# mikestir/webradio

Hardware: AMD Instinct MI355X
Metric: complex Msamples/sec (node), 256-ch DDC+NFM demod (higher is better)
Workload: dtype f32

## Files before the change

webradio_amd/csrc/wr_capi_internal.h:

```cpp
#ifndef WR_CAPI_INTERNAL_H
#define WR_CAPI_INTERNAL_H

#include "wr_internal.h"

#include <cstdarg>
#include <cstdio>
#include <cstdlib>
#include <cstring>
#include <new>
#include <atomic>
#include <chrono>
#include <map>
#include <mutex>
#include <vector>

#define HIP_TRY(expr)                                                                    \
	do {                                                                                 \
		hipError_t e_ = (expr);                                                          \
		if (e_ != hipSuccess)                                                            \
			return wrc_fail(WR_ERR_HIP, "%s: %s (%s:%d)", #expr, hipGetErrorString(e_),  \
			                __FILE__, __LINE__);                                         \
	} while (0)


// ... 130 lines not shown
	std::vector<hipEvent_t> ev;
	size_t ev_used;
	double prof_ms;
	unsigned int prof_n;
	struct RingSlot {
		float *host = nullptr;
		size_t cap = 0;
		hipEvent_t done = nullptr;
		size_t stride = 0, frames = 0;
		unsigned int slots = 0;
		unsigned long long seq = 0;
		unsigned int stream_wait = 0;
		unsigned long long stream_gen = 0;
	};
	std::vector<RingSlot> ring;
	unsigned int ring_head = 0, ring_count = 0;
	bool ring_held = false;
	unsigned long long ring_overruns = 0;
	unsigned long long submit_seq = 0;
	bool defer_post = true;
	unsigned int coalesce = 1;
	const float *held_base = nullptr;
	size_t held_frames = 0, held_each = 0;
	unsigned int held_count = 0;
	std::mutex ring_lock;
	struct Stream {
		bool enabled = false;
		bool host_bytes = false;
		bool live = false;
		bool unchecked = false;
		WrStreamCtl *ctl = nullptr;
		WrStreamDesc *desc = nullptr;
		WrStreamDev *sdev = nullptr;
		float *ring = nullptr;
		size_t ring_floats = 0;
		Group *g = nullptr;
		unsigned int count = 0;
		size_t nframes = 0;
		bool u8 = false;
		int parity0 = 0;
		size_t k1 = 0, k2 = 0;
		unsigned long long gen = 0;
		unsigned long long blocks = 0;
		std::chrono::steady_clock::time_point last_bell;
		const float *last_iq = nullptr;
		uint8_t *raw[4] = {nullptr, nullptr, nullptr, nullptr};
		size_t raw_cap = 0;
		unsigned long long raw_next = 0;
		unsigned long long raw_gen[4] = {0, 0, 0, 0};
		unsigned int raw_idx[4] = {0, 0, 0, 0};
		hipEvent_t raw_ev = nullptr;
		bool ext = false;
		bool up_pending = false;
		unsigned long long host_blocks = 0;
		unsigned long long long_blocks = 0;
	} stream;
};

struct wr_spectrum {
	wr_dev *dev;
	unsigned int n, hop;
	unsigned int ch;
	WrFftPlan plan;
	float *stage;
	size_t stage_cap;
	size_t pending;
// ... 66 lines not shown
```

webradio_amd/csrc/wr_internal.h:

```cpp
#ifndef WR_INTERNAL_H_
#define WR_INTERNAL_H_

#include <hip/hip_runtime.h>
#include <stddef.h>
#include <stdint.h>

#include "webradio_amd.h"

#define WR_HIST      (WR_FIR_LENGTH - 1)
#define WR_LANES     64
#define WR_SPLIT_N   256
#define WR_MAX_DEVICES 64
#define WR_TAPSETS   4

int         wrc_fail(int code, const char *fmt, ...) __attribute__((format(printf, 2, 3)));
int         wrc_dev_index(const wr_dev *dev);
hipStream_t wrc_dev_stream(const wr_dev *dev);
int         wrc_tuner_launch_mark(wr_tuner *t, hipEvent_t *ev);

void     wrd_sin_table(float *table);
void     wrd_sin_table_rounded(float *table);
int      wrd_phase_step(int if_hz, unsigned int input_rate);
unsigned wrd_lowpass_maxbin(unsigned int fir_length, unsigned int passband, unsigned int input_rate);
void     wrd_lowpass_design(unsigned int fir_length, unsigned int passband, unsigned int input_rate, float *coeff);
// ... 130 lines not shown
	unsigned int pad;
};
struct WrStreamCtl {
	volatile unsigned int ready;
	volatile unsigned int stop;
	volatile unsigned int pad0[14];
	volatile unsigned int done;
	volatile unsigned int final_blocks;
	volatile unsigned int err;
	volatile unsigned int self_closed;
	volatile unsigned int long_blocks;
	volatile unsigned int pad1[11];
};
#define WR_STREAM_SHARDS 16u
struct WrStreamDev {
	unsigned int ready, stop;
	unsigned long long beat;
	unsigned int ready_up;
	unsigned int pad0[27];
	unsigned long long progress;
	unsigned int drain_from;
	unsigned int pad1[29];
	unsigned int post_done[WR_STREAM_MAXJ];
	unsigned int post_fine[WR_STREAM_MAXJ];
	unsigned int post_ticket[WR_STREAM_MAXJ];
	unsigned int ddc_done[WR_STREAM_MAXJ][WR_STREAM_SHARDS][32];
	WrStreamDesc desc[WR_STREAM_MAXJ];
	unsigned long long cur[WR_STREAM_MAXJ + 1u];
};
struct WrStreamArgs {
	WrStreamCtl        *ctl;
	const WrStreamDesc *desc_host;
	WrStreamDev        *sdev;
	unsigned long long  idle_ticks;
	unsigned long long  wait_ticks;
	unsigned int        n_ddc, n_post;
	unsigned long long *tl;
	unsigned long long  cur0, audio0;
	unsigned long long  nframes;
	unsigned int        k1, d1, is_u8;
	unsigned int        ext;
	unsigned int        slots, groups;
	unsigned long long  gmap0, gmap1;
	unsigned int        kslow;
	unsigned int        kmax;
	const float        *hist;
	float              *hist_next;
	const unsigned int *phase, *step;
	unsigned int       *phase_next;
	const float        *hist_cs, *hist_lo;
	float              *hist_cs_next, *hist_lo_next;
	const int          *flags;
	const float        *taps1, *rot, *taps1u;
	const int          *tapsel;
	const float        *table, *hi_cs, *lo_cs;
	float              *ring;
	float              *audio_bufs[4];
	WrPostArgs          post;
	unsigned int        drain_run, drain_ntiles;
	const float        *prev_iq[2];
	float              *dem[2];
	int                 parity0;
	unsigned int        one_filter;
};
#define WR_STREAM_ERR_WAIT   1u
hipError_t wrk_stream_geometry(unsigned int d2, unsigned int groups, unsigned int kmax, bool one_filter, unsigned int nseg,
                               int num_cus, unsigned int *n_ddc, unsigned int *n_post);
hipError_t wrk_tuner_stream(hipStream_t st, const WrStreamArgs &A, void *ev_start, void *ev_stop);

struct WrFftPlan {
	unsigned int n;
	unsigned int channels;
	unsigned int n1, n2;
	float *tw_n;
	float *tw_sub;
	float *window;
	float *window_p1;
	float *work;
	size_t work_frames;
};
hipError_t wrk_fft_frames(hipStream_t st, const WrFftPlan &P, const float *iq, size_t hop,
                          size_t nframes_fft, float *bins_out , float *db_out );

hipError_t wrk_fft_cols(hipStream_t st, const WrFftPlan &P, const float *iq, unsigned int S, unsigned int cols, size_t first,
                        float *db, int num_cus );

size_t     wrk_chan_levels_work(unsigned int cols, size_t k1);
hipError_t wrk_chan_levels(hipStream_t st, const float *iq, size_t S, unsigned int cols, size_t k1, unsigned int d2, size_t k2,
                           const float *squelch, float *work, const float **out);

struct WrAgcPar {
	float        target;
// ... 26 lines not shown
```

webradio_amd/csrc/wr_stream_kernel.inc:

```

__device__ __forceinline__ unsigned int st_rfl(unsigned int v) { return __builtin_amdgcn_readfirstlane(v); }
__device__ __forceinline__ unsigned int st_ld(const unsigned int *p)
{
	return st_rfl(__hip_atomic_load(p, __ATOMIC_RELAXED, __HIP_MEMORY_SCOPE_AGENT));
}
__device__ __forceinline__ unsigned long long st_ld64(const unsigned long long *p)
{
	const unsigned long long v = __hip_atomic_load(p, __ATOMIC_RELAXED, __HIP_MEMORY_SCOPE_AGENT);
	return ((unsigned long long)st_rfl((unsigned int)(v >> 32)) << 32) | st_rfl((unsigned int)v);
}
__device__ __forceinline__ unsigned int st_ld_sys(const volatile unsigned int *p)
{
	return st_rfl(__hip_atomic_load((const unsigned int *)p, __ATOMIC_RELAXED, __HIP_MEMORY_SCOPE_SYSTEM));
}
__device__ __forceinline__ void st_st_sys(volatile unsigned int *p, unsigned int v)
{
	__hip_atomic_store((unsigned int *)p, v, __ATOMIC_RELAXED, __HIP_MEMORY_SCOPE_SYSTEM);
}

__device__ __forceinline__ unsigned int st_ddc_ready(const WrStreamArgs &S)
{
	return st_rfl((unsigned int)__hip_atomic_load(&S.sdev->progress, __ATOMIC_RELAXED, __HIP_MEMORY_SCOPE_AGENT));
}
__device__ __forceinline__ unsigned int st_post_ready(const WrStreamArgs &S)
{
	return st_rfl((unsigned int)(__hip_atomic_load(&S.sdev->progress, __ATOMIC_RELAXED, __HIP_MEMORY_SCOPE_AGENT) >> 32));
}

__device__ __forceinline__ void stream_fail(const WrStreamArgs &S)
{
	st_st_sys(&S.ctl->err, WR_STREAM_ERR_WAIT);
	__hip_atomic_store(&S.sdev->stop, 1u, __ATOMIC_RELAXED, __HIP_MEMORY_SCOPE_AGENT);
// ... 26 lines not shown
			if (now - t0 > S.wait_ticks && now >= beat && now - beat > S.wait_ticks) {
				stream_fail(S);
				if (r > known)
					known = r;
				closed = true;
				return false;
			}
		}
		__builtin_amdgcn_s_sleep(20);
	}
}

__device__ __forceinline__ bool stream_wait_count(const WrStreamArgs &S, const unsigned int *p, unsigned int target)
{
	if (st_ld(p) >= target)
		return true;
	const unsigned long long t0 = __builtin_amdgcn_s_memrealtime();
	unsigned int spins = 0;
	for (;;) {
		__builtin_amdgcn_s_sleep(20);
		if (st_ld(p) >= target)
			return true;
		if ((++spins & 63u) == 0u) {
			if (__builtin_amdgcn_s_memrealtime() - t0 > S.wait_ticks) {
				stream_fail(S);
				return false;
			}
			if (st_ld_sys(&S.ctl->err))
				return false;
		}
	}
}

#define STREAM_DRAIN_BLOCKS 2u
__device__ __forceinline__ void stream_watch(const WrStreamArgs &S)
{
	const unsigned int lane = threadIdx.x & 63u;
	__builtin_amdgcn_s_setprio(3);
	const unsigned int units = S.k1 * S.groups;
	unsigned int known = 1, jd = 0, jp = 0;
	unsigned int df = 0;
	unsigned int nlong = 0;
	bool closed = false;
	unsigned long long t_last = __builtin_amdgcn_s_memrealtime();
#ifdef STREAM_TL
	if ((threadIdx.x & 63u) == 0 && S.tl)
		S.tl[6999u * 8u + 0u] = t_last;
#endif
	for (;;) {
		bool moved = false;
		auto look = [&]() __attribute__((always_inline)) {
			const unsigned int r = st_ld(&S.sdev->ready);
			if (r > known)
				known = r;
			if (st_ld(&S.sdev->stop)) {
				const unsigned int f = st_ld(&S.sdev->ready);
				if (f > known)
					known = f;
				closed = true;
				const unsigned int from = known >= STREAM_DRAIN_BLOCKS ? known - STREAM_DRAIN_BLOCKS : 0u;
				df = (jd > from ? jd : from) + 1u;
				__hip_atomic_store(&S.sdev->drain_from, df, __ATOMIC_RELAXED, __HIP_MEMORY_SCOPE_AGENT);
				__builtin_amdgcn_fence(__ATOMIC_RELEASE, "agent");
			}
		};
		if (!closed && (jd >= known || jp >= known))
			look();
		if (jd < known && jd < WR_STREAM_MAXJ) {
			unsigned int v = 0;
			if (lane < WR_STREAM_SHARDS)
				v = __hip_atomic_load(&S.sdev->ddc_done[jd][lane][0], __ATOMIC_RELAXED, __HIP_MEMORY_SCOPE_AGENT);
#pragma unroll
			for (int o = 8; o >= 1; o >>= 1)
				v += __shfl_xor(v, o, 64);
			if (st_rfl(v) >= units) {
				{
					unsigned int fine = 1u;
					if (S.drain_run != S.post.run) {
						if (!closed)
							look();
						fine = (df && jd + 1u >= df) ? 1u : known >= jd + 3u ? 0u : 1u;
					}
					__hip_atomic_store(&S.sdev->post_fine[jd], fine, __ATOMIC_RELAXED, __HIP_MEMORY_SCOPE_AGENT);
					if (!fine && lane == 0)
						st_st_sys(&S.ctl->long_blocks, ++nlong);
					asm volatile("s_waitcnt vmcnt(0)" ::: "memory");
				}
				++jd;
				__hip_atomic_store(&S.sdev->progress, ((unsigned long long)jp << 32) | jd, __ATOMIC_RELAXED, __HIP_MEMORY_SCOPE_AGENT);
				moved = true;
#ifdef STREAM_TL
				if (lane == 0 && S.tl && jd <= 256u)
					S.tl[(7000u + jd - 1u) * 8u + 0u] = __builtin_amdgcn_s_memrealtime();
#endif
			}
		}
		if (jp < jd && st_ld(&S.sdev->post_done[jp]) >= (st_ld(&S.sdev->post_fine[jp]) ? S.drain_ntiles : S.post.ntiles) * S.post.groups) {
			++jp;
			__hip_atomic_store(&S.sdev->progress, ((unsigned long long)jp << 32) | jd, __ATOMIC_RELAXED, __HIP_MEMORY_SCOPE_AGENT);
			if (lane == 0)
				st_st_sys(&S.ctl->done, jp);
			moved = true;
#ifdef STREAM_TL
			if (lane == 0 && S.tl && jp <= 256u)
				S.tl[(7000u + jp - 1u) * 8u + 1u] = __builtin_amdgcn_s_memrealtime();
#endif
		}
		if (closed && jp >= known)
			return;
		const unsigned long long now = __builtin_amdgcn_s_memrealtime();
		if (moved) {
			t_last = now;
		} else {
			if ((jd < known || jp < jd) && now - t_last > S.wait_ticks) {
				stream_fail(S);
				return;
			}
			if (closed && st_ld_sys(&S.ctl->err))
				return;
			__builtin_amdgcn_s_sleep(4);
		}
	}
}

__device__ __forceinline__ void stream_bell(const WrStreamArgs &S)
{
	if (threadIdx.x >= 64u && threadIdx.x < 128u) {
		stream_watch(S);
		return;
	}
	if (threadIdx.x != 0)
		return;
	__builtin_amdgcn_s_setprio(3);
	unsigned int seen = 1;
	__hip_atomic_store(&S.sdev->desc[0].cur, S.cur0, __ATOMIC_RELAXED, __HIP_MEMORY_SCOPE_AGENT);
	__hip_atomic_store(&S.sdev->desc[0].audio_host, S.audio0, __ATOMIC_RELAXED, __HIP_MEMORY_SCOPE_AGENT);
	__hip_atomic_store(&S.sdev->cur[1], S.cur0, __ATOMIC_RELAXED, __HIP_MEMORY_SCOPE_AGENT);
	asm volatile("s_waitcnt vmcnt(0)" ::: "memory");
	unsigned long long t_last = __builtin_amdgcn_s_memrealtime();
	for (;;) {
		__hip_atomic_store(&S.sdev->beat, (unsigned long long)__builtin_amdgcn_s_memrealtime(), __ATOMIC_RELAXED,
		                   __HIP_MEMORY_SCOPE_AGENT);
		const unsigned int s = st_ld_sys(&S.ctl->stop);
		unsigned int r = st_ld_sys(&S.ctl->ready);
		{
			const unsigned int ru = st_ld(&S.sdev->ready_up);
			if (ru > r)
				r = ru;
		}
		if (r > WR_STREAM_MAXJ)
			r = WR_STREAM_MAXJ;
		if (r > seen) {
			for (unsigned int j = seen; j < r; ++j) {
				const unsigned long long c = __hip_atomic_load(&S.desc_host[j].cur, __ATOMIC_RELAXED, __HIP_MEMORY_SCOPE_SYSTEM);
				const unsigned long long a = __hip_atomic_load(&S.desc_host[j].audio_host, __ATOMIC_RELAXED, __HIP_MEMORY_SCOPE_SYSTEM);
				__hip_atomic_store(&S.sdev->desc[j].cur, c, __ATOMIC_RELAXED, __HIP_MEMORY_SCOPE_AGENT);
				__hip_atomic_store(&S.sdev->cur[j + 1u], c, __ATOMIC_RELAXED, __HIP_MEMORY_SCOPE_AGENT);
				__hip_atomic_store(&S.sdev->desc[j].audio_host, a, __ATOMIC_RELAXED, __HIP_MEMORY_SCOPE_AGENT);
			}
			asm volatile("s_waitcnt vmcnt(0)" ::: "memory");
			__hip_atomic_store(&S.sdev->ready, r, __ATOMIC_RELAXED, __HIP_MEMORY_SCOPE_AGENT);
			seen = r;
			t_last = __builtin_amdgcn_s_memrealtime();
		}
		if (s || st_ld(&S.sdev->stop)) {
			asm volatile("s_waitcnt vmcnt(0)" ::: "memory");
			__hip_atomic_store(&S.sdev->stop, 1u, __ATOMIC_RELAXED, __HIP_MEMORY_SCOPE_AGENT);
			return;
		}
		if (seen >= WR_STREAM_MAXJ || __builtin_amdgcn_s_memrealtime() - t_last > S.idle_ticks) {
			if (seen < WR_STREAM_MAXJ)
				st_st_sys(&S.ctl->self_closed, 1u);
			asm volatile("s_waitcnt vmcnt(0)" ::: "memory");
			__hip_atomic_store(&S.sdev->stop, 1u, __ATOMIC_RELAXED, __HIP_MEMORY_SCOPE_AGENT);
			return;
		}
		__builtin_amdgcn_s_sleep(40);
	}
}

template <unsigned int PD2, unsigned int TS, unsigned int NSEG>
__device__ __forceinline__ void stream_post(const WrStreamArgs &S, const unsigned int p, v2f *lds, const bool helper)
{
	constexpr unsigned int D2 = PD2 ? PD2 : 1u;
	constexpr unsigned int NEED = (POST_TK - 1u) * D2 + WR_FIR_LENGTH * NSEG;
	wave_prio(3u);
	if (threadIdx.x >= POST_THREADS)
		return;
	const unsigned int wave = st_rfl(threadIdx.x >> 6);
	const unsigned int waves_per_wg = POST_THREADS / 64u;
#ifdef STREAM_TL
	if (threadIdx.x == 0 && S.tl && !helper)
		S.tl[(6000u + p) * 8u + 7u] = 12345ull;
#endif

	const unsigned int n_bnd = (S.kslow * S.groups + waves_per_wg - 1u) / waves_per_wg;
	if (!helper && p < n_bnd) {
		const unsigned long long c0 = S.cur0;
		ddc_body<WR_NCO_ROTATE, true, PD2>(S.is_u8 ? nullptr : (const float2 *)c0, S.is_u8 ? (const uchar2 *)c0 : nullptr,
		                                   (const float2 *)S.hist, (float2 *)S.hist_next, (size_t)S.nframes, (size_t)S.k1, S.d1,
		                                   S.slots, S.groups, S.phase, S.step, (const float2 *)S.hist_cs, S.flags, S.phase_next,
		                                   (float2 *)S.hist_cs_next, (const float2 *)S.hist_lo, (float2 *)S.hist_lo_next, S.taps1,
		                                   (const float4 *)S.rot, S.taps1u, S.tapsel, TS == 1u ? 1u : S.kmax, (float2 *)S.ring, S.table,
		                                   (const float2 *)S.hi_cs, (const float2 *)S.lo_cs, S.n_ddc, S.post, S.gmap0, S.gmap1, 0,
		                                   S.kslow, 0x40000000u, 0u, 0u, lds, DDC_ROLE_BOUNDARY);
		const unsigned int ub = p * waves_per_wg + wave;
		asm volatile("s_waitcnt vmcnt(0)" ::: "memory");
		if (ub / S.groups < S.kslow && (threadIdx.x & 63u) == 0u)
			__hip_atomic_fetch_add(&S.sdev->ddc_done[0][ub % WR_STREAM_SHARDS][0], 1u, __ATOMIC_RELAXED, __HIP_MEMORY_SCOPE_AGENT);
		wave_prio(3u);
		__syncthreads();
	}

	float *stage = (float *)lds;
	float *tile = stage + NEED * 64u;
	int *modes = (int *)(tile + POST_TK * 65u);
	unsigned int *sh = (unsigned int *)(modes + 64);
	const unsigned int tasks = S.post.ntiles * S.post.groups;
	unsigned int known = 1;
	bool closed = false;
	unsigned int j = 0;
	if (helper) {
		if (threadIdx.x == 0)
			sh[6] = st_ld(&S.sdev->drain_from);
		__syncthreads();
		const unsigned int df = sh[6];
		if (!df)
// ... 10 lines not shown
		if (threadIdx.x == 0) {
			bool ok = j < WR_STREAM_MAXJ && stream_wait_ready(S, j, known, closed);
			if (ok) {
				const unsigned int need_hi = j >= 4u ? j - 3u : 0u;
				const unsigned long long t0 = __builtin_amdgcn_s_memrealtime();
				unsigned int spins = 0;
				for (;;) {
					const unsigned long long pg = st_ld64(&S.sdev->progress);
					if ((unsigned int)pg >= j + 1u && (unsigned int)(pg >> 32) >= need_hi)
						break;
					if ((++spins & 63u) == 0u) {
						if (__builtin_amdgcn_s_memrealtime() - t0 > S.wait_ticks) {
							stream_fail(S);
							ok = false;
							break;
						}
						if (st_ld_sys(&S.ctl->err)) {
							ok = false;
							break;
						}
					}
					__builtin_amdgcn_s_sleep(20);
				}
			}
			unsigned long long ah = 0;
			unsigned int drain = helper ? 1u : 0u;
			if (ok) {
				ah = j ? st_ld64(&S.sdev->desc[j].audio_host) : S.audio0;
				__builtin_amdgcn_fence(__ATOMIC_ACQUIRE, "agent");
				if (!helper) {
					const unsigned int df = st_ld(&S.sdev->drain_from);
					drain = (df && j + 1u >= df) ? 1u : 0u;
				}
				sh[7] = (helper || drain) ? 1u : st_ld(&S.sdev->post_fine[j]);
			}
			sh[5] = drain;
			sh[0] = ok ? 1u : 0u;
			sh[1] = (unsigned int)ah;
			sh[2] = (unsigned int)(ah >> 32);
			sh[3] = known;
		}
		__syncthreads();
		const bool go = sh[0] != 0u;
		const unsigned long long ah = ((unsigned long long)sh[2] << 32) | sh[1];
		known = sh[3];
		if (!go)
			break;
		WrPostArgs A = S.post;
		A.chan_iq = S.ring + (size_t)(j % WR_STREAM_RING) * S.k1 * S.slots * 2u;
		A.chan_prev = j ? S.ring + (size_t)((j - 1u) % WR_STREAM_RING) * S.k1 * S.slots * 2u : nullptr;
		A.prev_iq = S.prev_iq[S.parity0];
		A.dem_hist = S.dem[S.parity0];
		A.audio_host = (float *)ah;
		A.audio = S.audio_bufs[j & 3u];
#ifdef STREAM_TL
		const unsigned long long pt1 = __builtin_amdgcn_s_memtime();
		if (threadIdx.x == 0 && S.tl && !helper && p < 4u && j < 256u)
			S.tl[(7300u + j) * 8u + p * 2u] = __builtin_amdgcn_s_memrealtime();
#endif
		const bool drain = sh[5] != 0u;
		if (sh[7] != 0u) {
			A.run = S.drain_run;
			A.ntiles = S.drain_ntiles;
		}
		const unsigned int tasks_j = A.ntiles * A.groups;
		unsigned int mine = 0;
		const unsigned int rot = (unsigned int)(((unsigned long long)j * tasks) % S.n_post);
		for (unsigned int t = p >= rot ? p - rot : p + S.n_post - rot;; t += S.n_post) {
			if (drain) {
				if (threadIdx.x == 0)
					sh[4] = __hip_atomic_fetch_add(&S.sdev->post_ticket[j], 1u, __ATOMIC_RELAXED, __HIP_MEMORY_SCOPE_AGENT);
				__syncthreads();
				t = sh[4];
			}
			if (t >= tasks_j)
				break;
			post_role<D2, false, NSEG>(A, t % A.ntiles, t / A.ntiles, stage, tile, modes);
			__syncthreads();
			++mine;
		}
		if (threadIdx.x == 0 && mine) {
			if (ah)
				__builtin_amdgcn_fence(__ATOMIC_RELEASE, "");
			else
				__builtin_amdgcn_fence(__ATOMIC_RELEASE, "agent");
			asm volatile("s_waitcnt vmcnt(0)" ::: "memory");
			__hip_atomic_fetch_add(&S.sdev->post_done[j], mine, __ATOMIC_RELAXED, __HIP_MEMORY_SCOPE_AGENT);
		}
#ifdef STREAM_TL
		if (threadIdx.x == 0 && S.tl && !helper && p < 4u && j < 256u)
			S.tl[(7300u + j) * 8u + p * 2u + 1u] = __builtin_amdgcn_s_memrealtime();
		if (threadIdx.x == 0) {
			const unsigned long long pt3 = __builtin_amdgcn_s_memtime();
			pt_wait += pt1 - pt0;
			pt_sync += pt3 - pt1;
			++pt_n;
// ... 331 lines not shown
	return nseg == 1u || nseg == 2u || (nseg == 4u && d2 <= STREAM_NSEG4_MAX_D2);
}
template <unsigned int PD2, class F>
static hipError_t with_stream_nseg(unsigned int nseg, F &&f)
{
	if (nseg == 1u)
		return f(std::integral_constant<unsigned int, 1u>());
	if (nseg == 2u)
		return f(std::integral_constant<unsigned int, 2u>());
	if constexpr (PD2 <= STREAM_NSEG4_MAX_D2)
		if (nseg == 4u)
			return f(std::integral_constant<unsigned int, 4u>());
	return hipErrorInvalidValue;
}

template <unsigned int PD2, unsigned int NG, unsigned int TS, unsigned int NSEG>
static hipError_t stream_allow_lds(size_t lds)
{
	static bool attr_done[WR_MAX_DEVICES];
	if (lds <= 64 * 1024)
		return hipSuccess;
	return allow_lds((const void *)k_tuner_stream<PD2, NG, TS, NSEG>, stream_lds_bytes(PD2, TS, NSEG), attr_done);
}

template <unsigned int PD2, unsigned int NG, unsigned int TS, unsigned int NSEG>
static hipError_t stream_occupancy(size_t lds, int *per_cu)
{
	hipError_t e = stream_allow_lds<PD2, NG, TS, NSEG>(lds);
	if (e != hipSuccess)
		return e;
	return hipOccupancyMaxActiveBlocksPerMultiprocessor(per_cu, k_tuner_stream<PD2, NG, TS, NSEG>, (int)(DDC_ROTATE_WAVES * 64u), lds);
}

hipError_t wrk_stream_geometry(unsigned int d2, unsigned int groups, unsigned int kmax, bool one_filter, unsigned int nseg,
                               int num_cus, unsigned int *n_ddc, unsigned int *n_post)
{
	*n_ddc = *n_post = 0;
	if (!wrk_tuner_post_supported(d2) || !stream_nseg_supported(d2, nseg) || !groups || groups > 16u || !kmax ||
	    kmax > WR_TAPSETS)
		return hipSuccess;
	unsigned int ng, ts;
	stream_shape(groups, kmax, one_filter, &ng, &ts);
	const size_t lds = stream_lds_bytes(d2, ts == 1u ? 1u : kmax, nseg);
	int per_cu = 0;
	hipError_t e = with_post_d2(d2, [&](auto D2) {
		constexpr unsigned int PD2 = decltype(D2)::value;
		return with_stream_nseg<PD2>(nseg, [&](auto NS) {
			constexpr unsigned int NSEG = decltype(NS)::value;
			return ts != 1u ? stream_occupancy<PD2, 1, WR_TAPSETS, NSEG>(lds, &per_cu)
			       : ng == 1u ? stream_occupancy<PD2, 1, 1, NSEG>(lds, &per_cu)
			                  : stream_occupancy<PD2, 2, 1, NSEG>(lds, &per_cu);
		});
	});
	if (e != hipSuccess)
		return e;
	if (per_cu > 3)
		per_cu = 3;
	if (per_cu < 2)
		return hipSuccess;
	*n_ddc = (unsigned int)(per_cu - 1) * (unsigned int)num_cus;
	*n_post = (unsigned int)num_cus - 4u;
	return hipSuccess;
}

template <unsigned int PD2, unsigned int NG, unsigned int TS, unsigned int NSEG>
static hipError_t launch_stream(hipStream_t st, const WrStreamArgs &A, void *ev_start, void *ev_stop)
{
	const size_t lds = stream_lds_bytes(PD2, TS == 1u ? 1u : A.kmax, NSEG);
	hipError_t e = stream_allow_lds<PD2, NG, TS, NSEG>(lds);
	if (e != hipSuccess)
		return e;
	const unsigned int grid = A.n_ddc + A.n_post + 1u;
	if (ev_start || ev_stop) {
		hipExtLaunchKernelGGL((k_tuner_stream<PD2, NG, TS, NSEG>), dim3(grid), dim3(DDC_ROTATE_WAVES * 64u), (uint32_t)lds, st,
		                      (hipEvent_t)ev_start, (hipEvent_t)ev_stop, 0u, A);
		return hipGetLastError();
	}
	k_tuner_stream<PD2, NG, TS, NSEG><<<grid, DDC_ROTATE_WAVES * 64u, lds, st>>>(A);
	return hipGetLastError();
}

hipError_t wrk_tuner_stream(hipStream_t st, const WrStreamArgs &A0, void *ev_start, void *ev_stop)
{
	WrStreamArgs A = A0;
	if (!A.n_ddc || !A.n_post || !A.groups || A.groups > 16u || !A.k1)
		return hipErrorInvalidValue;
	const unsigned int min_run = stream_post_run(A.post.tiles, A.post.groups, A.n_post);
	A.post.run = min_run;
	if (min_run >= 2u && A.n_post >= 8u)
		A.post.run = stream_post_run(A.post.tiles, A.post.groups, A.n_post / 2u);
	while (A.post.run < 4u && A.post.run < A.post.tiles &&
	       ((A.post.tiles + A.post.run - 1u) / A.post.run) * A.post.groups > A.n_post / 4u &&
	       ((A.post.tiles + A.post.run - 1u) / A.post.run) * A.post.groups <= A.n_post / 2u)
		++A.post.run;
	A.post.ntiles = (A.post.tiles + A.post.run - 1u) / A.post.run;
	A.drain_run = min_run < A.post.run ? min_run : A.post.run;
	A.drain_ntiles = (A.post.tiles + A.drain_run - 1u) / A.drain_run;
	const unsigned int tasks = A.post.ntiles * A.post.groups;
	(void)tasks;
	if (!A.kmax || A.kmax > WR_TAPSETS)
		return hipErrorInvalidValue;
	unsigned int ng, ts;
	stream_shape(A.groups, A.kmax, A.one_filter != 0u, &ng, &ts);
	if ((size_t)A.n_ddc * DDC_ROTATE_WAVES < A.groups / ng)
		return hipErrorInvalidValue;
	if (A.k1 < WR_FIR_LENGTH * A.post.nseg)
		return hipErrorInvalidValue;
	return with_post_d2(A.post.d2, [&](auto D2) {
		constexpr unsigned int PD2 = decltype(D2)::value;
		return with_stream_nseg<PD2>(A.post.nseg, [&](auto NS) {
			constexpr unsigned int NSEG = decltype(NS)::value;
			return ts != 1u ? launch_stream<PD2, 1, WR_TAPSETS, NSEG>(st, A, ev_start, ev_stop)
			       : ng == 2u ? launch_stream<PD2, 2, 1, NSEG>(st, A, ev_start, ev_stop)
			                  : launch_stream<PD2, 1, 1, NSEG>(st, A, ev_start, ev_stop);
		});
	});
}
```

webradio_amd/csrc/wr_tuner_stream.hip:

```cpp
#include "wr_capi_internal.h"


static unsigned long long *g_stream_tl = nullptr;
extern "C" int wr_debug_stream_tl(unsigned long long *out, size_t n)
{
	if (!g_stream_tl)
		return 1;
	memcpy(out, g_stream_tl, n * sizeof(unsigned long long));
	return 0;
}

static std::mutex g_stream_mu;
static wr_tuner *g_stream_on[WR_MAX_DEVICES];

static void stream_raw_free(wr_tuner::Stream &s)
{
	for (uint8_t *&r : s.raw) {
		(void)hipFree(r);
		r = nullptr;
	}
	s.raw_cap = 0;
}

void wrc_stream_free(wr_tuner *t)
{
	wr_tuner::Stream &s = t->stream;
	(void)hipHostFree(s.ctl);
	(void)hipHostFree(s.desc);
	(void)hipFree(s.sdev);
	(void)hipFree(s.ring);
	stream_raw_free(s);
	if (s.raw_ev)
		(void)hipEventDestroy(s.raw_ev);
	s.raw_ev = nullptr;
	s.ctl = nullptr;
	s.desc = nullptr;
	s.sdev = nullptr;
	s.ring = nullptr;
	s.ring_floats = 0;
}

int wrc_stream_check(wr_tuner *t)
{
	wr_tuner::Stream &s = t->stream;
	if (!s.unchecked)
		return WR_OK;
	s.unchecked = false;
	s.long_blocks += s.ctl->long_blocks;
	s.ctl->long_blocks = 0;
	if (s.ctl->err)
		return wrc_fail(WR_ERR_HIP, "streaming launch: a wait inside the launch ran into its deadline (code %u)", s.ctl->err);
	if (s.ctl->final_blocks != s.count)
		return wrc_fail(WR_ERR_STATE, "streaming launch: %u blocks rung, %u processed%s", s.count, s.ctl->final_blocks,
		                s.ctl->self_closed ? " (the launch had closed itself: the doorbell was silent too long)" : "");
	return WR_OK;
}

bool wrc_stream_follows(const wr_tuner *t, size_t nframes, int where, bool u8)
{
	const wr_tuner::Stream &s = t->stream;
	if (!s.live || !s.enabled || where != WR_DEVICE || nframes != s.nframes || u8 != s.u8 || s.count >= WR_STREAM_MAXJ)
		return false;
	if (s.g->dirty)
		return false;
	const auto idle = std::chrono::steady_clock::now() - s.last_bell;
	return idle < std::chrono::milliseconds(WR_STREAM_STALE_MS);
}

int wrc_stream_bell(wr_tuner *t, const void *iq, bool behind_upload)
{
	wr_tuner::Stream &s = t->stream;
	const unsigned int j = s.count;
	const unsigned long long seq = t->submit_seq++;
	float *slot = wrc_stream_ring_entry(t, s.g, seq, s.k2, wrc_group_slots_used(s.g), j);
	s.desc[j].cur = (unsigned long long)(uintptr_t)iq;
	s.desc[j].audio_host = (unsigned long long)(uintptr_t)slot;
	s.desc[j].count = j + 1u;
	std::atomic_thread_fence(std::memory_order_release);
	if (behind_upload) {
		HIP_TRY(hipStreamWriteValue32(t->dev->up_stream, &s.sdev->ready_up, j + 1u, 0));
		s.up_pending = true;
	} else {
		if (s.up_pending) {
			HIP_TRY(hipStreamSynchronize(t->dev->up_stream));
			s.up_pending = false;
		}
		s.ctl->ready = j + 1u;
	}
	std::atomic_thread_fence(std::memory_order_seq_cst);
	s.count = j + 1u;
	++s.blocks;
	s.last_bell = std::chrono::steady_clock::now();
	return WR_OK;
}

int wrc_stream_open(wr_tuner *t, const void *iq, size_t nframes, bool u8, bool *took)
{
	*took = false;
	wr_tuner::Stream &s = t->stream;
	wr_dev *d = t->dev;
	if (t->nco_mode != WR_NCO_ROTATE || !t->defer_post || t->mark_launches || (t->keep_mask & (1u << WR_STAGE_DEMOD)))
		return WR_OK;
	Group *g = wrc_single_group(t);
	if (!g || g->l1 != WR_FIR_LENGTH || g->d1b || g->seek_pending || !wrk_tuner_post_supported(g->d2))
		return WR_OK;
	if (g->l2 != WR_FIR_LENGTH && g->l2 != 2u * WR_FIR_LENGTH && g->l2 != 4u * WR_FIR_LENGTH)
		return WR_OK;
	const unsigned int nseg = g->l2 / WR_FIR_LENGTH;
	if (nframes < (size_t)g->l2 * g->d1 || nframes % ((size_t)g->d1 * g->d2) || nframes / g->d1 > 0x3FFFFFFFu)
		return WR_OK;
	if (wrc_dev_bind(d))
		return WR_ERR_HIP;
	if (int rc = wrc_tuner_launch_held(t))
		return rc;
	if (g->dirty)
		if (int rc = wrc_group_upload(t, g))
			return rc;
	if (g->use_agc)
		return WR_OK;
	const unsigned int used = wrc_group_slots_used(g), groups = used / 64u;
	if (!groups || groups > 16u)
		return WR_OK;
	const unsigned long long used_mask = (1ull << groups) - 1ull;
	if ((g->fewsets_mask & used_mask) != used_mask)
		return WR_OK;
	unsigned int kmax = 1;
	for (unsigned int gi = 0; gi < groups; ++gi)
		if (g->nsets[gi] > kmax)
			kmax = g->nsets[gi];
	if (int rc = wrc_dev_settle_stream(d))
		return rc;
	{
		std::lock_guard<std::mutex> lk(g_stream_mu);
		if (d->device < 0 || d->device >= WR_MAX_DEVICES || (g_stream_on[d->device] && g_stream_on[d->device] != t))
			return WR_OK;
	}
	if (s.unchecked) {
		HIP_TRY(wrc_dev_stream_sync(d));
		if (int rc = wrc_stream_check(t))
			return rc;
	}
	if (g->post_pending)
		if (int rc = wrc_tuner_flush(t))
			return rc;
	const size_t k1 = nframes / g->d1, k2 = k1 / g->d2;
	unsigned int n_ddc = 0, n_post = 0;
	HIP_TRY(wrk_stream_geometry(g->d2, groups, kmax, g->one_filter, nseg, d->num_cus, &n_ddc, &n_post));
	if (!n_ddc || !n_post)
		return WR_OK;
	if (!s.ctl)
		HIP_TRY(hipHostMalloc((void **)&s.ctl, sizeof(WrStreamCtl), hipHostMallocMapped | hipHostMallocCoherent));
	if (!s.desc)
		HIP_TRY(hipHostMalloc((void **)&s.desc, sizeof(WrStreamDesc) * WR_STREAM_MAXJ, hipHostMallocMapped | hipHostMallocCoherent));
	if (!s.sdev)
		HIP_TRY(hipMalloc((void **)&s.sdev, sizeof(WrStreamDev)));
	const size_t ring_floats = (size_t)WR_STREAM_RING * k1 * g->slots * 2u;
	if (ring_floats > s.ring_floats) {
		HIP_TRY(wrc_dev_stream_sync(d));
		(void)hipFree(s.ring);
		s.ring = nullptr;
		s.ring_floats = 0;
		HIP_TRY(hipMalloc((void **)&s.ring, ring_floats * sizeof(float)));
		s.ring_floats = ring_floats;
	}
	void *ctl_dev = nullptr, *desc_dev = nullptr;
	HIP_TRY(hipHostGetDevicePointer(&ctl_dev, s.ctl, 0));
	HIP_TRY(hipHostGetDevicePointer(&desc_dev, s.desc, 0));
	hipStream_t st = d->stream;

	const WrTunerLaunch L = wrc_group_launch(t, g, u8 ? nullptr : (const float *)iq, u8 ? (const uint8_t *)iq : nullptr, nframes);

	WrStreamArgs A;
	memset(&A, 0, sizeof(A));
	A.ctl = (WrStreamCtl *)ctl_dev;
	A.desc_host = (const WrStreamDesc *)desc_dev;
	A.sdev = s.sdev;
	A.idle_ticks = (unsigned long long)WR_STREAM_IDLE_MS * 100000ull;
	A.wait_ticks = (unsigned long long)WR_STREAM_WAIT_MS * 100000ull;
	A.n_ddc = n_ddc;
	A.n_post = n_post;
	if (getenv("WR_STREAM_TL") && atoi(getenv("WR_STREAM_TL"))) {
		static unsigned long long *tlbuf = nullptr;
		if (!tlbuf)
			HIP_TRY(hipHostMalloc((void **)&tlbuf, 8192 * 8 * sizeof(unsigned long long), hipHostMallocMapped | hipHostMallocCoherent));
		memset(tlbuf, 0, 8192 * 8 * sizeof(unsigned long long));
		void *tld = nullptr;
		HIP_TRY(hipHostGetDevicePointer(&tld, tlbuf, 0));
		A.tl = (unsigned long long *)tld;
		g_stream_tl = tlbuf;
	}
	A.nframes = nframes;
	A.k1 = (unsigned int)k1;
	A.d1 = g->d1;
	A.is_u8 = u8 ? 1u : 0u;
	A.ext = s.ext ? 1u : 0u;
	A.slots = g->slots;
	A.groups = groups;
	for (unsigned int gi = 0; gi < groups; ++gi)
		(gi < 8u ? A.gmap0 : A.gmap1) |= (unsigned long long)gi << ((gi & 7u) * 8u);
	A.kslow = (WR_HIST + g->d1 - 1u) / g->d1;
	if (A.kslow > k1)
		A.kslow = (unsigned int)k1;
	A.hist = L.hist;
	A.hist_next = L.hist_next;
	A.phase = g->dev.phase[g->sp];
	A.step = g->dev.step;
	A.phase_next = g->dev.phase[g->sp ^ 1];
	A.hist_cs = g->dev.hist_cs[g->sp];
	A.hist_lo = g->dev.hist_lo[g->sp];
// ... 11 lines not shown
	for (int i = 0; i < 4; ++i)
		A.audio_bufs[i] = g->dev.audio_set[(g->audio_cur + i) & 3];
	A.post = wrk_post_args(L, g->dev);
	A.post.host_stride = k2;
	A.prev_iq[0] = g->dev.prev_iq[0];
	A.prev_iq[1] = g->dev.prev_iq[1];
	A.dem[0] = g->dev.dem[0];
	A.dem[1] = g->dev.dem[1];
	A.parity0 = g->parity;
	A.kmax = kmax;
	A.one_filter = g->one_filter ? 1u : 0u;

	++s.gen;
	s.g = g;
	s.count = 0;
	s.nframes = nframes;
	s.u8 = u8;
	s.parity0 = g->parity;
	s.k1 = k1;
	s.k2 = k2;
	s.last_iq = nullptr;
	const unsigned long long seq = t->submit_seq++;
	float *slot = wrc_stream_ring_entry(t, g, seq, k2, used, 0);
	s.ctl->ready = 1;
	s.ctl->stop = 0;
	s.ctl->done = 0;
	s.ctl->final_blocks = 0;
	s.ctl->long_blocks = 0;
	s.ctl->err = 0;
	s.ctl->self_closed = 0;
	s.desc[0].cur = (unsigned long long)(uintptr_t)iq;
	s.desc[0].audio_host = (unsigned long long)(uintptr_t)slot;
	std::atomic_thread_fence(std::memory_order_seq_cst);
	if (s.ext) {
		HIP_TRY(hipMemsetAsync(s.sdev, 0, offsetof(WrStreamDev, ready_up), st));
		const size_t after = offsetof(WrStreamDev, ready_up) + sizeof(unsigned int);
		HIP_TRY(hipMemsetAsync((char *)s.sdev + after, 0, offsetof(WrStreamDev, desc) - after, st));
	} else {
		HIP_TRY(hipMemsetAsync(s.sdev, 0, offsetof(WrStreamDev, desc), st));
	}
	A.cur0 = s.desc[0].cur;
	A.audio0 = s.desc[0].audio_host;

	void *ev0 = nullptr, *ev1 = nullptr;
	if (t->profiling && !(t->ev_used & 1))
		if (int rc = wrc_prof_pair_begin(t, &ev0, &ev1))
			return rc;
	HIP_TRY(wrk_tuner_stream(st, A, ev0, ev1));
	if (ev0)
		wrc_prof_pair_stamped(t);
	s.live = true;
	s.count = 1;
	++s.blocks;
	s.last_bell = std::chrono::steady_clock::now();
	d->streaming = t;
	{
		std::lock_guard<std::mutex> lk(g_stream_mu);
		g_stream_on[d->device] = t;
	}
	*took = true;
	return WR_OK;
}

int wrc_stream_host_u8(wr_tuner *t, const uint8_t *bytes, size_t nframes, bool *took)
{
	*took = false;
	wr_tuner::Stream &s = t->stream;
	wr_dev *d = t->dev;
	if (wrc_dev_bind(d))
		return WR_ERR_HIP;
	if (!wrc_host_mapped(bytes))
		return WR_OK;
	const size_t need = nframes * 2;
	if (need <= WR_STREAM_HOST_MIN_BYTES)
		return WR_OK;
	const bool follows = s.live && s.ext && wrc_stream_follows(t, nframes, WR_DEVICE, true);
	if (need > s.raw_cap) {
		if (int rc = wrc_stream_close(t))
			return rc;
		HIP_TRY(wrc_dev_stream_sync(d));
		if (d->up_stream)
			HIP_TRY(hipStreamSynchronize(d->up_stream));
		stream_raw_free(s);
		for (uint8_t *&r : s.raw)
			HIP_TRY(hipMalloc((void **)&r, need));
		s.raw_cap = need;
	}
	const unsigned int slot = (unsigned int)(s.raw_next & 3u);
	const unsigned int through = s.raw_idx[slot] + 2u < s.count ? s.raw_idx[slot] + 2u : s.count;
	if ((s.live || s.unchecked) && s.raw_gen[slot] == s.gen && s.ctl->done < through) {
		const auto t0 = std::chrono::steady_clock::now();
		while (s.ctl->done < through && !s.ctl->err)
			if (std::chrono::steady_clock::now() - t0 > std::chrono::milliseconds(4 * WR_STREAM_WAIT_MS))
				return wrc_fail(WR_ERR_HIP, "streaming launch: block %u did not finish", s.raw_idx[slot] + 1u);
	}
	{
		std::lock_guard<std::mutex> up_guard(*d->upload_lock);
		if (int rc = wrc_dev_up_stream(d))
			return rc;
		HIP_TRY(hipMemcpyAsync(s.raw[slot], bytes, need, hipMemcpyHostToDevice, d->up_stream));
		if (int rc = wrc_upload_mark_locked(d, d->up_stream))
			return rc;
	}
	if (follows) {
		s.raw_gen[slot] = s.gen;
		s.raw_idx[slot] = s.count;
		++s.raw_next;
		++s.host_blocks;
		t->last_staging = 3;
		*took = true;
		return wrc_stream_bell(t, s.raw[slot], true);
	}
	if (int rc = wrc_stream_close(t))
		return rc;
	if (!s.raw_ev)
		HIP_TRY(hipEventCreateWithFlags(&s.raw_ev, hipEventDisableTiming));
	if (!s.sdev)
		HIP_TRY(hipMalloc((void **)&s.sdev, sizeof(WrStreamDev)));
	HIP_TRY(hipStreamWriteValue32(d->up_stream, &s.sdev->ready_up, 0u, 0));
	HIP_TRY(hipEventRecord(s.raw_ev, d->up_stream));
	HIP_TRY(hipStreamWaitEvent(d->stream, s.raw_ev, 0));
	s.ext = true;
	bool opened = false;
	if (int rc = wrc_stream_open(t, s.raw[slot], nframes, true, &opened))
		return rc;
	s.raw_gen[slot] = opened ? s.gen : 0;
	s.raw_idx[slot] = 0;
	++s.raw_next;
	*took = true;
	if (opened) {
		++s.host_blocks;
		t->last_staging = 3;
		return WR_OK;
	}
	s.ext = false;
	t->last_staging = 1;
	return wrc_tuner_submit_now(t, s.raw[slot], nframes, WR_DEVICE, true);
}

int wrc_stream_close(wr_tuner *t)
{
	wr_tuner::Stream &s = t->stream;
	if (!s.live)
		return WR_OK;
	if (s.up_pending) {
		HIP_TRY(hipStreamSynchronize(t->dev->up_stream));
		s.ctl->ready = s.count;
		s.up_pending = false;
	}
	std::atomic_thread_fence(std::memory_order_seq_cst);
	s.ctl->stop = 1;
	std::atomic_thread_fence(std::memory_order_seq_cst);
	s.live = false;
	s.unchecked = true;
	if (t->dev->streaming == t)
		t->dev->streaming = nullptr;
	{
		std::lock_guard<std::mutex> lk(g_stream_mu);
		if (g_stream_on[t->dev->device] == t)
			g_stream_on[t->dev->device] = nullptr;
	}
	Group *g = s.g;
	const unsigned int J = s.count;
	for (Group *x : t->groups)
		if (x != g)
			x->last_k1 = x->last_k2 = 0;
	g->sp ^= 1;
	g->last_parity = s.parity0;
	g->parity = s.parity0 ^ 1;
	g->last_k1 = s.k1;
	g->last_k2 = s.k2;
	g->last_demod_kept = false;
	s.last_iq = s.ring + (size_t)((J - 1u) % WR_STREAM_RING) * s.k1 * g->slots * 2u;
	g->audio_cur = (int)((g->audio_cur + (J - 1u)) & 3u);
	g->dev.audio = g->dev.audio_set[g->audio_cur];
	t->in_par ^= 1;
	wrc_advance_phases(t, (unsigned long long)s.nframes * J);
	t->submitted = true;
	return WR_OK;
}

extern "C" int wr_tuner_set_streaming(wr_tuner *t, int enable)
{
	if (!t)
		return wrc_fail(WR_ERR_ARG, "tuner is NULL");
	if (wrc_dev_bind(t->dev))
		return WR_ERR_HIP;
// ... 36 lines not shown
```

Before: 117,500.

## Double-buffer stream device state, zero next buffer in-kernel, cache geometry queries

Keeps two device-side stream control blocks and has the post workers zero the inactive one while the current launch runs. The next open can then skip the memset launches when that buffer is known clean. It also caches the occupancy query per geometry key and caches the mapped host pointers. A third, smaller post run size is added for the final blocks of a closed stream, which shortens the tail. Together this lowers per-open host overhead and drain latency, at the cost of more state to keep consistent: clean flags, buffer swaps on close, and the ext guard on ready_up.

```diff
diff --git a/webradio_amd/csrc/wr_capi_internal.h b/webradio_amd/csrc/wr_capi_internal.h
--- a/webradio_amd/csrc/wr_capi_internal.h
+++ b/webradio_amd/csrc/wr_capi_internal.h
@@ -186,6 +186,10 @@
 		WrStreamCtl *ctl = nullptr;
 		WrStreamDesc *desc = nullptr;
 		WrStreamDev *sdev = nullptr;
+		WrStreamDev *sdev2[2] = {nullptr, nullptr};
+		bool sdev_clean[2] = {false, false};
+		unsigned int sdev_cur = 0;
+		void *ctl_dev = nullptr, *desc_dev = nullptr;
 		float *ring = nullptr;
 		size_t ring_floats = 0;
 		Group *g = nullptr;
diff --git a/webradio_amd/csrc/wr_internal.h b/webradio_amd/csrc/wr_internal.h
--- a/webradio_amd/csrc/wr_internal.h
+++ b/webradio_amd/csrc/wr_internal.h
@@ -186,6 +186,7 @@
 	WrStreamCtl        *ctl;
 	const WrStreamDesc *desc_host;
 	WrStreamDev        *sdev;
+	WrStreamDev        *sdev_next;
 	unsigned long long  idle_ticks;
 	unsigned long long  wait_ticks;
 	unsigned int        n_ddc, n_post;
@@ -211,7 +212,7 @@
 	float              *ring;
 	float              *audio_bufs[4];
 	WrPostArgs          post;
-	unsigned int        drain_run, drain_ntiles;
+	unsigned int        drain_run, last_run;
 	const float        *prev_iq[2];
 	float              *dem[2];
 	int                 parity0;
diff --git a/webradio_amd/csrc/wr_stream_kernel.inc b/webradio_amd/csrc/wr_stream_kernel.inc
--- a/webradio_amd/csrc/wr_stream_kernel.inc
+++ b/webradio_amd/csrc/wr_stream_kernel.inc
@@ -1,3 +1,7 @@
+
+#include <mutex>
+#include <utility>
+#include <vector>
 
 __device__ __forceinline__ unsigned int st_rfl(unsigned int v) { return __builtin_amdgcn_readfirstlane(v); }
 __device__ __forceinline__ unsigned int st_ld(const unsigned int *p)
@@ -90,7 +94,9 @@
 	}
 }
 
-#define STREAM_DRAIN_BLOCKS 2u
+#ifndef STREAM_TAIL_BLOCKS
+#define STREAM_TAIL_BLOCKS 2u
+#endif
 __device__ __forceinline__ void stream_watch(const WrStreamArgs &S)
 {
 	const unsigned int lane = threadIdx.x & 63u;
@@ -99,6 +105,10 @@
 	unsigned int known = 1, jd = 0, jp = 0;
 	unsigned int df = 0;
 	unsigned int nlong = 0;
+	const unsigned int nt_short = (S.post.tiles + S.drain_run - 1u) / S.drain_run, nt_last = (S.post.tiles + S.last_run - 1u) / S.last_run;
+	auto ntiles_of = [&](unsigned int run) __attribute__((always_inline)) {
+		return run == S.post.run ? S.post.ntiles : run == S.drain_run ? nt_short : nt_last;
+	};
 	bool closed = false;
 	unsigned long long t_last = __builtin_amdgcn_s_memrealtime();
 #ifdef STREAM_TL
@@ -116,7 +126,7 @@
 				if (f > known)
 					known = f;
 				closed = true;
-				const unsigned int from = known >= STREAM_DRAIN_BLOCKS ? known - STREAM_DRAIN_BLOCKS : 0u;
+				const unsigned int from = known >= STREAM_TAIL_BLOCKS ? known - STREAM_TAIL_BLOCKS : 0u;
 				df = (jd > from ? jd : from) + 1u;
 				__hip_atomic_store(&S.sdev->drain_from, df, __ATOMIC_RELAXED, __HIP_MEMORY_SCOPE_AGENT);
 				__builtin_amdgcn_fence(__ATOMIC_RELEASE, "agent");
@@ -133,14 +143,15 @@
 				v += __shfl_xor(v, o, 64);
 			if (st_rfl(v) >= units) {
 				{
-					unsigned int fine = 1u;
-					if (S.drain_run != S.post.run) {
-						if (!closed)
-							look();
-						fine = (df && jd + 1u >= df) ? 1u : known >= jd + 3u ? 0u : 1u;
-					}
-					__hip_atomic_store(&S.sdev->post_fine[jd], fine, __ATOMIC_RELAXED, __HIP_MEMORY_SCOPE_AGENT);
-					if (!fine && lane == 0)
+					if (!closed)
+						look();
+					unsigned int run;
+					if (closed)
+						run = jd + 1u >= known ? S.last_run : jd + STREAM_TAIL_BLOCKS >= known ? S.drain_run : S.post.run;
+					else
+						run = known >= jd + 3u ? S.post.run : S.drain_run;
+					__hip_atomic_store(&S.sdev->post_fine[jd], run, __ATOMIC_RELAXED, __HIP_MEMORY_SCOPE_AGENT);
+					if (run == S.post.run && S.post.run != S.drain_run && lane == 0)
 						st_st_sys(&S.ctl->long_blocks, ++nlong);
 					asm volatile("s_waitcnt vmcnt(0)" ::: "memory");
 				}
@@ -153,7 +164,7 @@
 #endif
 			}
 		}
-		if (jp < jd && st_ld(&S.sdev->post_done[jp]) >= (st_ld(&S.sdev->post_fine[jp]) ? S.drain_ntiles : S.post.ntiles) * S.post.groups) {
+		if (jp < jd && st_ld(&S.sdev->post_done[jp]) >= ntiles_of(st_ld(&S.sdev->post_fine[jp])) * S.post.groups) {
 			++jp;
 			__hip_atomic_store(&S.sdev->progress, ((unsigned long long)jp << 32) | jd, __ATOMIC_RELAXED, __HIP_MEMORY_SCOPE_AGENT);
 			if (lane == 0)
@@ -202,7 +213,7 @@
 		const unsigned int s = st_ld_sys(&S.ctl->stop);
 		unsigned int r = st_ld_sys(&S.ctl->ready);
 		{
-			const unsigned int ru = st_ld(&S.sdev->ready_up);
+			const unsigned int ru = S.ext ? st_ld(&S.sdev->ready_up) : 0u;
 			if (ru > r)
 				r = ru;
 		}
@@ -251,6 +262,14 @@
 	if (threadIdx.x == 0 && S.tl && !helper)
 		S.tl[(6000u + p) * 8u + 7u] = 12345ull;
 #endif
+	if (!helper && S.sdev_next) {
+		unsigned int *z = (unsigned int *)S.sdev_next;
+		constexpr unsigned int nz = (unsigned int)(offsetof(WrStreamDev, desc) / sizeof(unsigned int));
+		constexpr unsigned int skip = (unsigned int)(offsetof(WrStreamDev, ready_up) / sizeof(unsigned int));
+		for (unsigned int i = p * POST_THREADS + threadIdx.x; i < nz; i += S.n_post * POST_THREADS)
+			if (i != skip)
+				z[i] = 0u;
+	}
 
 	const unsigned int n_bnd = (S.kslow * S.groups + waves_per_wg - 1u) / waves_per_wg;
 	if (!helper && p < n_bnd) {
@@ -327,7 +346,7 @@
 					const unsigned int df = st_ld(&S.sdev->drain_from);
 					drain = (df && j + 1u >= df) ? 1u : 0u;
 				}
-				sh[7] = (helper || drain) ? 1u : st_ld(&S.sdev->post_fine[j]);
+				sh[7] = st_ld(&S.sdev->post_fine[j]);
 			}
 			sh[5] = drain;
 			sh[0] = ok ? 1u : 0u;
@@ -354,9 +373,9 @@
 			S.tl[(7300u + j) * 8u + p * 2u] = __builtin_amdgcn_s_memrealtime();
 #endif
 		const bool drain = sh[5] != 0u;
-		if (sh[7] != 0u) {
-			A.run = S.drain_run;
-			A.ntiles = S.drain_ntiles;
+		if (sh[7] != A.run) {
+			A.run = sh[7];
+			A.ntiles = (A.tiles + A.run - 1u) / A.run;
 		}
 		const unsigned int tasks_j = A.ntiles * A.groups;
 		unsigned int mine = 0;
@@ -754,18 +773,47 @@
 	return hipOccupancyMaxActiveBlocksPerMultiprocessor(per_cu, k_tuner_stream<PD2, NG, TS, NSEG>, (int)(DDC_ROTATE_WAVES * 64u), lds);
 }
 
+static unsigned long long stream_geometry_key(int device, unsigned int d2, unsigned int groups, unsigned int kmax, bool one_filter,
+                                           unsigned int nseg)
+{
+	unsigned int ng, ts;
+	stream_shape(groups, kmax, one_filter, &ng, &ts);
+	const unsigned int nset = ts == 1u ? 1u : kmax;
+	return ((unsigned long long)(unsigned int)device << 32) | ((unsigned long long)d2 << 24) | ((unsigned long long)nseg << 16) |
+	       ((unsigned long long)nset << 8) | ((unsigned long long)ng << 4) | (ts == 1u ? 0ull : 1ull);
+}
+
 hipError_t wrk_stream_geometry(unsigned int d2, unsigned int groups, unsigned int kmax, bool one_filter, unsigned int nseg,
                                int num_cus, unsigned int *n_ddc, unsigned int *n_post)
 {
 	*n_ddc = *n_post = 0;
 	if (!wrk_tuner_post_supported(d2) || !stream_nseg_supported(d2, nseg) || !groups || groups > 16u || !kmax ||
 	    kmax > WR_TAPSETS)
+		return hipSuccess;
+	if (num_cus < 8)
 		return hipSuccess;
 	unsigned int ng, ts;
 	stream_shape(groups, kmax, one_filter, &ng, &ts);
 	const size_t lds = stream_lds_bytes(d2, ts == 1u ? 1u : kmax, nseg);
 	int per_cu = 0;
-	hipError_t e = with_post_d2(d2, [&](auto D2) {
+	int device = 0;
+	hipError_t e = hipGetDevice(&device);
+	if (e != hipSuccess)
+		return e;
+	static std::mutex mu;
+	static std::vector<std::pair<unsigned long long, int>> seen;
+	const unsigned long long key = stream_geometry_key(device, d2, groups, kmax, one_filter, nseg);
+	bool hit = false;
+	{
+		std::lock_guard<std::mutex> lk(mu);
+		for (const auto &kv : seen)
+			if (kv.first == key) {
+				per_cu = kv.second;
+				hit = true;
+			}
+	}
+	if (!hit)
+	e = with_post_d2(d2, [&](auto D2) {
 		constexpr unsigned int PD2 = decltype(D2)::value;
 		return with_stream_nseg<PD2>(nseg, [&](auto NS) {
 			constexpr unsigned int NSEG = decltype(NS)::value;
@@ -776,6 +824,10 @@
 	});
 	if (e != hipSuccess)
 		return e;
+	if (!hit) {
+		std::lock_guard<std::mutex> lk(mu);
+		seen.emplace_back(key, per_cu);
+	}
 	if (per_cu > 3)
 		per_cu = 3;
 	if (per_cu < 2)
@@ -817,7 +869,9 @@
 		++A.post.run;
 	A.post.ntiles = (A.post.tiles + A.post.run - 1u) / A.post.run;
 	A.drain_run = min_run < A.post.run ? min_run : A.post.run;
-	A.drain_ntiles = (A.post.tiles + A.drain_run - 1u) / A.drain_run;
+	A.last_run = stream_post_run(A.post.tiles, A.post.groups, A.n_ddc + A.n_post);
+	if (A.last_run > A.drain_run)
+		A.last_run = A.drain_run;
 	const unsigned int tasks = A.post.ntiles * A.post.groups;
 	(void)tasks;
 	if (!A.kmax || A.kmax > WR_TAPSETS)
diff --git a/webradio_amd/csrc/wr_tuner_stream.hip b/webradio_amd/csrc/wr_tuner_stream.hip
--- a/webradio_amd/csrc/wr_tuner_stream.hip
+++ b/webradio_amd/csrc/wr_tuner_stream.hip
@@ -22,12 +22,28 @@
 	s.raw_cap = 0;
 }
 
+static int stream_sdev_alloc(wr_tuner::Stream &s)
+{
+	for (int i = 0; i < 2; ++i)
+		if (!s.sdev2[i]) {
+			HIP_TRY(hipMalloc((void **)&s.sdev2[i], sizeof(WrStreamDev)));
+			s.sdev_clean[i] = false;
+		}
+	s.sdev = s.sdev2[s.sdev_cur];
+	return WR_OK;
+}
+
 void wrc_stream_free(wr_tuner *t)
 {
 	wr_tuner::Stream &s = t->stream;
 	(void)hipHostFree(s.ctl);
 	(void)hipHostFree(s.desc);
-	(void)hipFree(s.sdev);
+	for (int i = 0; i < 2; ++i) {
+		(void)hipFree(s.sdev2[i]);
+		s.sdev2[i] = nullptr;
+		s.sdev_clean[i] = false;
+	}
+	s.ctl_dev = s.desc_dev = nullptr;
 	(void)hipFree(s.ring);
 	stream_raw_free(s);
 	if (s.raw_ev)
@@ -48,6 +64,8 @@
 	s.unchecked = false;
 	s.long_blocks += s.ctl->long_blocks;
 	s.ctl->long_blocks = 0;
+	if (s.ctl->err || s.ctl->final_blocks != s.count)
+		s.sdev_clean[0] = s.sdev_clean[1] = false;
 	if (s.ctl->err)
 		return wrc_fail(WR_ERR_HIP, "streaming launch: a wait inside the launch ran into its deadline (code %u)", s.ctl->err);
 	if (s.ctl->final_blocks != s.count)
@@ -94,9 +112,19 @@
 	return WR_OK;
 }
 
+#ifdef STREAM_TL
+#define OPEN_STAMP(i) (open_us[i] = std::chrono::duration<double, std::micro>(std::chrono::steady_clock::now() - open_t0).count())
+#else
+#define OPEN_STAMP(i) ((void)0)
+#endif
+
 int wrc_stream_open(wr_tuner *t, const void *iq, size_t nframes, bool u8, bool *took)
 {
 	*took = false;
+#ifdef STREAM_TL
+	const auto open_t0 = std::chrono::steady_clock::now();
+	double open_us[6] = {0, 0, 0, 0, 0, 0};
+#endif
 	wr_tuner::Stream &s = t->stream;
 	wr_dev *d = t->dev;
 	if (t->nco_mode != WR_NCO_ROTATE || !t->defer_post || t->mark_launches || (t->keep_mask & (1u << WR_STAGE_DEMOD)))
@@ -145,15 +173,17 @@
 			return rc;
 	const size_t k1 = nframes / g->d1, k2 = k1 / g->d2;
 	unsigned int n_ddc = 0, n_post = 0;
+	OPEN_STAMP(0);
 	HIP_TRY(wrk_stream_geometry(g->d2, groups, kmax, g->one_filter, nseg, d->num_cus, &n_ddc, &n_post));
 	if (!n_ddc || !n_post)
 		return WR_OK;
+	OPEN_STAMP(1);
 	if (!s.ctl)
 		HIP_TRY(hipHostMalloc((void **)&s.ctl, sizeof(WrStreamCtl), hipHostMallocMapped | hipHostMallocCoherent));
 	if (!s.desc)
 		HIP_TRY(hipHostMalloc((void **)&s.desc, sizeof(WrStreamDesc) * WR_STREAM_MAXJ, hipHostMallocMapped | hipHostMallocCoherent));
-	if (!s.sdev)
-		HIP_TRY(hipMalloc((void **)&s.sdev, sizeof(WrStreamDev)));
+	if (int rc = stream_sdev_alloc(s))
+		return rc;
 	const size_t ring_floats = (size_t)WR_STREAM_RING * k1 * g->slots * 2u;
 	if (ring_floats > s.ring_floats) {
 		HIP_TRY(wrc_dev_stream_sync(d));
@@ -163,18 +193,21 @@
 		HIP_TRY(hipMalloc((void **)&s.ring, ring_floats * sizeof(float)));
 		s.ring_floats = ring_floats;
 	}
-	void *ctl_dev = nullptr, *desc_dev = nullptr;
-	HIP_TRY(hipHostGetDevicePointer(&ctl_dev, s.ctl, 0));
-	HIP_TRY(hipHostGetDevicePointer(&desc_dev, s.desc, 0));
+	if (!s.ctl_dev)
+		HIP_TRY(hipHostGetDevicePointer(&s.ctl_dev, s.ctl, 0));
+	if (!s.desc_dev)
+		HIP_TRY(hipHostGetDevicePointer(&s.desc_dev, s.desc, 0));
 	hipStream_t st = d->stream;
+	OPEN_STAMP(2);
 
 	const WrTunerLaunch L = wrc_group_launch(t, g, u8 ? nullptr : (const float *)iq, u8 ? (const uint8_t *)iq : nullptr, nframes);
 
 	WrStreamArgs A;
 	memset(&A, 0, sizeof(A));
-	A.ctl = (WrStreamCtl *)ctl_dev;
-	A.desc_host = (const WrStreamDesc *)desc_dev;
+	A.ctl = (WrStreamCtl *)s.ctl_dev;
+	A.desc_host = (const WrStreamDesc *)s.desc_dev;
 	A.sdev = s.sdev;
+	A.sdev_next = s.sdev2[s.sdev_cur ^ 1u];
 	A.idle_ticks = (unsigned long long)WR_STREAM_IDLE_MS * 100000ull;
 	A.wait_ticks = (unsigned long long)WR_STREAM_WAIT_MS * 100000ull;
 	A.n_ddc = n_ddc;
@@ -252,7 +285,9 @@
 	s.desc[0].cur = (unsigned long long)(uintptr_t)iq;
 	s.desc[0].audio_host = (unsigned long long)(uintptr_t)slot;
 	std::atomic_thread_fence(std::memory_order_seq_cst);
-	if (s.ext) {
+	OPEN_STAMP(3);
+	if (s.sdev_clean[s.sdev_cur]) {
+	} else if (s.ext) {
 		HIP_TRY(hipMemsetAsync(s.sdev, 0, offsetof(WrStreamDev, ready_up), st));
 		const size_t after = offsetof(WrStreamDev, ready_up) + sizeof(unsigned int);
 		HIP_TRY(hipMemsetAsync((char *)s.sdev + after, 0, offsetof(WrStreamDev, desc) - after, st));
@@ -261,6 +296,7 @@
 	}
 	A.cur0 = s.desc[0].cur;
 	A.audio0 = s.desc[0].audio_host;
+	OPEN_STAMP(4);
 
 	void *ev0 = nullptr, *ev1 = nullptr;
 	if (t->profiling && !(t->ev_used & 1))
@@ -269,6 +305,14 @@
 	HIP_TRY(wrk_tuner_stream(st, A, ev0, ev1));
 	if (ev0)
 		wrc_prof_pair_stamped(t);
+	OPEN_STAMP(5);
+#ifdef STREAM_TL
+	if (getenv("WR_STREAM_TL") && atoi(getenv("WR_STREAM_TL")) == 2)
+		fprintf(stderr, "stream open [us]: checks %.1f geometry %.1f allocations+pointers %.1f arguments %.1f fill %.1f launch %.1f\n", open_us[0],
+		        open_us[1] - open_us[0], open_us[2] - open_us[1], open_us[3] - open_us[2], open_us[4] - open_us[3], open_us[5] - open_us[4]);
+#endif
+	s.sdev_clean[s.sdev_cur] = false;
+	s.sdev_clean[s.sdev_cur ^ 1u] = true;
 	s.live = true;
 	s.count = 1;
 	++s.blocks;
@@ -335,8 +379,8 @@
 		return rc;
 	if (!s.raw_ev)
 		HIP_TRY(hipEventCreateWithFlags(&s.raw_ev, hipEventDisableTiming));
-	if (!s.sdev)
-		HIP_TRY(hipMalloc((void **)&s.sdev, sizeof(WrStreamDev)));
+	if (int rc = stream_sdev_alloc(s))
+		return rc;
 	HIP_TRY(hipStreamWriteValue32(d->up_stream, &s.sdev->ready_up, 0u, 0));
 	HIP_TRY(hipEventRecord(s.raw_ev, d->up_stream));
 	HIP_TRY(hipStreamWaitEvent(d->stream, s.raw_ev, 0));
@@ -373,6 +417,8 @@
 	std::atomic_thread_fence(std::memory_order_seq_cst);
 	s.live = false;
 	s.unchecked = true;
+	s.sdev_cur ^= 1u;
+	s.sdev = s.sdev2[s.sdev_cur];
 	if (t->dev->streaming == t)
 		t->dev->streaming = nullptr;
 	{
```

Measured after the change: 117,300. About the same (-0.1%).
